# cityflow-project/CityFlow

Measured on NVIDIA H100. Metric: vehicle_steps_per_sec, higher is better.
Workload: dtype f64

## Files before the change

### cityflow_b200/csrc/device_phases_a.cuh

```cuda
#pragma once

namespace cfb {

__device__ __forceinline__ void blkSet(const View &V, int slot, int val) {
    if (val == -2) {
        V.blk[slot] = -1;
        V.delStep[slot] = V.ctrl->step;
    } else {
        V.blk[slot] = val;
    }
    if (V.blkUpd) {
        const int i = atomicAdd(&V.ctrl->nBlkUpd, 1);
        if (i < V.blkUpdCap) V.blkUpd[1 + i] = make_int2(slot, val); else atomicOr(&V.ctrl->error, ERR_MOVER_OVERFLOW);
    }
}

__device__ __forceinline__ int planAt(const View &V, int plan, int idx) { return V.planData[V.planBeg[plan] + idx]; }
__device__ __forceinline__ void foeTerms(const View &V, Notify &n, int foeLinkW);

__device__ void headSearch(const View &V, int d, double dis, int nextDrv, int planIdx, const DTmpl &T, int myLane,
                           int &outLeader, double &outGap) {
    int leader = -1;
    double gap = 0;
    double x = V.drvLength[d] - dis;
    int nd = nextDrv;
    for (int i = 0;; ++i) {
        if (i > 0) nd = V.planData[planIdx + 1 + i];
        if (nd < 0) break;
        if (nd >= V.nLanes) {
            const int sl = V.llStartLane[nd - V.nLanes];
            for (int q = V.laneOutBeg[sl]; q < V.laneOutBeg[sl + 1]; ++q) {
                const Tail t = V.tail[V.nLanes + V.laneOutLinks[q]];
                if (t.pos >= 0) {
                    double candGap = x + t.dis - t.len;
                    if (leader < 0 || candGap < gap) {
                        leader = t.pos;
                        gap = candGap;
                    }
                }
            }
            if (leader >= 0) break;
        } else {
            Tail t = V.tail[nd];
            if (myLane >= 0 && nd > myLane && (V.inserted[nd] & 1)) {
                const int c = V.count[nd] - 1;
                if (c > 0) {
                    const int tp = V.off[nd] + c - 1;
                    t.pos = tp;
                    t.dis = V.kin[tp].x;
                    t.len = V.tmpl[V.ids[tp].y].len;
                } else {
                    t.pos = -1;
                }
            }
            if (t.pos >= 0) {
                leader = t.pos;
                gap = x + t.dis - t.len;
                break;
            }
        }
        x += V.drvLength[nd];
        if (x > T.approachDist) break;
    }
    outLeader = leader;
    if (leader >= 0) outGap = gap;
}

// ... 177 lines not shown
        }
        if (valid && owner >= 0) {
            Notify n;
            n.dist = ndist;
            n.pos = owner;
            n.epoch = epoch;
            foeTerms(V, n, linkW);
            V.notify[V.lcIdx[cb + k]] = n;
            const int peer = V.lcPeer[cb + k];
            const int foeLink = V.csLink[V.lcIdx[cb + k] ^ 1];
            const int bit = peer - V.llCrossBeg[foeLink];
            atomicOr(&V.foeMask[foeLink * V.maskWords + (bit >> 5)], 1u << (bit & 31));
        }
    }
}

__device__ __forceinline__ void phase_notify(const View &V, const int bid, const int nblk) {
    const int lane = threadIdx.x & 31, tile = lane >> 4, tl = lane & 15;
    const int warp = (bid * blockDim.x + threadIdx.x) >> 5;
    const int nWarps = (nblk * blockDim.x) >> 5;
    const int cpar = V.par;
    const int nAct = V.ctrl->nAct[cpar];
    const int epoch = V.ctrl->step + 1;
    for (int w0 = 2 * warp; w0 < nAct; w0 += 2 * nWarps) {
        const int w = w0 + tile;
        int la = -1, lb = -1;
        if (w < nAct) {
            const int d = V.actList[cpar][w];
            if (d >= V.nLanes) {
                la = d - V.nLanes;
            } else if (V.count[d] > 0) {
                const int c = V.count[d], base = V.off[d];
                if ((V.inserted[d] & 2) && tl == 0 && !V.lcOn) {
                    const int4 idv = V.ids[base];
                    int ld = -1;
                    double g = 0;
                    headSearch(V, d, 0.0, idv.w, V.nav[base].x, V.tmpl[idv.y], d, ld, g);
                    V.leader[base] = ld;
                    if (ld >= 0) V.gap[base] = g;
                    if (V.lcOn && ld >= 0) V.lc.slot[idv.x].gap = g;
                }
                const int prev = V.nav[base + c - 1].y;
                if (prev >= V.nLanes && V.count[prev] == 0 && (!V.owned || V.owned[prev] == 1)) la = prev - V.nLanes;
                const int nx = V.ids[base].w;
                if (nx >= V.nLanes && V.count[nx] == 0 && nx - V.nLanes != la) lb = nx - V.nLanes;
                if (la < 0) { la = lb; lb = -1; }
            }
        }
        notifyLink(V, la, tl, epoch);
        if (__ballot_sync(0xffffffffu, lb >= 0)) notifyLink(V, lb, tl, epoch);
    }
    for (int w0 = 2 * warp; w0 < V.nBoundOut; w0 += 2 * nWarps) {
        const int w = w0 + tile;
        int l = -1;
        if (w < V.nBoundOut) {
            const Tail t = V.tail[V.boundOut[w]];
            if (t.pos >= 0 && t.prev >= V.nLanes && V.owned[t.prev] == 1 && V.count[t.prev] == 0) l = t.prev - V.nLanes;
        }
        notifyLink(V, l, tl, epoch);
    }
}

}
```

### cityflow_b200/csrc/device_phases_b.cuh

```cuda
#pragma once

namespace cfb {

static_assert(ENT_CAP <= 16, "k_move sorts a drivable's entrants inside one 16-lane tile");
__device__ __forceinline__ void phase_move(const View &V, const int bid, const int nblk) {
    const int lane = threadIdx.x & 31, tile = lane >> 4, tl = lane & 15, tb = lane & 16;
    const int cpar = V.par, npar = cpar ^ 1;
    const int nAct = V.ctrl->nAct[cpar];
    const int nTot = nAct + V.ctrl->nExtra;
    __shared__ int sTot[16];
    __shared__ int sBaseVeh, sBaseAct;
    const int tib = threadIdx.x >> 4, tpb = blockDim.x >> 4;
    for (int w0 = bid * tpb; w0 < nTot; w0 += nblk * tpb) {
        const int w = w0 + tib;
        int d = -1, n = 0, mIn = 0, base = 0, cap = 0;
        if (w < nTot) {
            d = w < nAct ? V.actList[cpar][w] : V.extraList[w - nAct];
            n = V.count[d];
            mIn = V.entCnt[d];
            base = V.off[d];
            cap = V.off[d + 1] - base;
        }
        const int nMax = max(n, __shfl_xor_sync(0xffffffffu, n, 16));
        int nsurv = 0;
// ... 115 lines not shown
            }
            V.tail[d] = t;
        }
        if (tl == 0) sTot[tib] = total;
        __syncthreads();
        if (threadIdx.x == 0) {
            int sv = 0, sa = 0;
            for (int k = 0; k < tpb; ++k) { sv += sTot[k]; sa += sTot[k] > 0; }
            sBaseVeh = sv ? atomicAdd(&V.ctrl->nVeh[npar], sv) : 0;
            sBaseAct = sa ? atomicAdd(&V.ctrl->nAct[npar], sa) : 0;
        }
        __syncthreads();
        if (total > 0) {
            int offV = sBaseVeh, offA = sBaseAct;
            for (int k = 0; k < tib; ++k) { offV += sTot[k]; offA += sTot[k] > 0; }
            if (tl == 0) V.actList[npar][offA] = d;
            for (int k = tl; k < total; k += 16)
                if (offV + k < V.vehCap) V.vehList[npar][offV + k] = make_int2(base + k, k == 0 ? (d | HEAD_BIT) : d);
        }
        __syncthreads();
    }
}

__device__ __forceinline__ void phase_leader(const View &V, const int bid, const int nblk) {
    const int gtid = bid * blockDim.x + threadIdx.x;
    const int lane = threadIdx.x & 31;
    const int warp = gtid >> 5;
    const int nWarps = (nblk * blockDim.x) >> 5;
    const int npar = V.par ^ 1;
    const int nAct = V.ctrl->nAct[npar];
    if (gtid == 0) {
        V.ctrl->step += 1;
        V.ctrl->epoch += 1;
        V.ctrl->vehicleSteps += (unsigned long long) (long long) V.ctrl->active;
        if (V.hostMirror) {
            volatile int *m = V.hostMirror;
            m[1] = V.ctrl->active;
            m[2] = V.ctrl->error;
            m[3] = V.ctrl->ties;
            __threadfence_system();
            m[0] = V.ctrl->epoch;
        }
    }
    if (!V.rl) {
        for (int in = gtid; in < V.nInter; in += nblk * blockDim.x) {
            if (V.interVirtual[in]) continue;
            double rem = V.remain[in] - V.dt;
            int cur = V.curPhase[in];
            const int pb = V.interPhaseBeg[in], nph = V.interPhaseBeg[in + 1] - pb;
            while (rem <= 0.0) {
                cur = (cur + 1) % nph;
                rem += V.phaseTime[pb + cur];
            }
            V.remain[in] = rem;
            V.curPhase[in] = cur;
        }
    }
    const int stride = nblk * blockDim.x;
    (void) lane; (void) warp; (void) nWarps;
    for (int w = gtid; w < nAct; w += stride) {
        const int d = V.actList[npar][w];
        const int p = V.off[d];
        const int4 idv = V.ids[p];
        int ld = -1;
        double g = 0;
        headSearch(V, d, V.kin[p].x, idv.w, V.nav[p].x, V.tmpl[idv.y], -1, ld, g);
        V.leader[p] = ld;
        if (ld >= 0) V.gap[p] = g;
        if (V.lcOn && ld >= 0) V.lc.slot[idv.x].gap = g;
    }
}

}
```

### cityflow_b200/csrc/device_sim.cu

```cuda
#include <cuda_runtime.h>
#include <cooperative_groups.h>

#include <algorithm>
#include <chrono>
#include <climits>
#include <cstdio>
#include <cstdlib>
#include <cstring>
#include <stdexcept>
#include <string>
#include <vector>

#include "device_sim.h"
#include "partition.h"
#include "shard.h"

namespace cfb {
namespace cg = cooperative_groups;

#define CFB_CUDA(x)                                                                                  \
    do {                                                                                             \
        cudaError_t e_ = (x);                                                                        \
        if (e_ != cudaSuccess)                                                                       \
            throw std::runtime_error(std::string("cityflow_b200 CUDA error: ") + cudaGetErrorString(e_) + \
// ... 4 lines not shown
#include "device_view.cuh"
#include "device_image.cuh"
#include "device_layout.cuh"
#include "device_phases_a.cuh"
namespace cfb {
__device__ __forceinline__ void pdlEnter() {
    asm volatile("griddepcontrol.wait;" ::: "memory");
    asm volatile("griddepcontrol.launch_dependents;" ::: "memory");
}
__global__ void __launch_bounds__(256) k_ingest(View V) { pdlEnter(); phase_ingest(V, blockIdx.x, gridDim.x); }
__global__ void __launch_bounds__(256) k_notify(View V) { pdlEnter(); phase_notify(V, blockIdx.x, gridDim.x); }

}
#include "device_control.cuh"
namespace cfb {

__global__ void __launch_bounds__(256, 4) k_control(View V) { pdlEnter(); phase_control(V, blockIdx.x, gridDim.x); }

}
#include "device_phases_b.cuh"
namespace cfb {
__global__ void __launch_bounds__(256) k_move(View V) { pdlEnter(); phase_move(V, blockIdx.x, gridDim.x); }
__global__ void __launch_bounds__(256) k_leader(View V) { pdlEnter(); phase_leader(V, blockIdx.x, gridDim.x); }

__global__ void __launch_bounds__(256, 4) k_step(View V) {
    cg::grid_group grid = cg::this_grid();
    phase_ingest(V, blockIdx.x, gridDim.x);
    grid.sync();
    phase_notify(V, blockIdx.x, gridDim.x);
    grid.sync();
    phase_control(V, blockIdx.x, gridDim.x);
    grid.sync();
    phase_move(V, blockIdx.x, gridDim.x);
    grid.sync();
    phase_leader(V, blockIdx.x, gridDim.x);
}

}
#include "device_shard.cuh"
namespace cfb {

__global__ void k_mask_counts(View V, int *out) {
    const int i = blockIdx.x * blockDim.x + threadIdx.x;
    if (i == 0) out[0] = V.ctrl->active;
    if (i < V.nLanes) out[1 + i] = (!V.owned || V.owned[i] == 1) ? V.count[i] : 0;
}
// ... 228 lines not shown
    cudaEvent_t obsReady = nullptr, obsConsumed = nullptr;
    cudaEvent_t actReady = nullptr, actTaken = nullptr;
    bool hPhaseStale = false;
    std::vector<cudaEvent_t> stepEv;
    size_t stepEvUsed = 0;
    DevBuf<unsigned char> flushBuf;
    KernelTimes times;
    cudaEvent_t shardEv[SHARD_PHASES + 1] = {};
    double shardMs[SHARD_PHASES] = {};
    long long shardTimedSteps = 0;

    DevBuf<LcSlot> lcSlot;
    DevBuf<int> lcLaneRoad, lcRouteLastRoad, lcScratch;
    bool lcSerial = false;
    DevBuf<int> lcSegIdx, lcPosDrv, lcSegBeg, lcLaneIdx, lcLaneRoadN, lcPlanRoute, lcPlanRoadPos, lcLanePlanRoad,
        lcLanePlanBeg, lcLanePlanId, lcCand, lcInvolved, lcSpare, lcPrio;
    DevBuf<double> lcSegStart, lcLaneWidth;
    DevBuf<int2> lcShadowLog;
    DevBuf<LcCtrl> lcCtrl;
    LcCtrl *hLcCtrl = nullptr;
    int lcSpareCap = 0;
    int slotCap = 0;
    int numSMs = 132;
    int gridNotify = 0, gridMove = 0, gridLeader = 0, gridControl = 0;
    bool mirrorStale = false;
    bool usePdl = true;
    bool useGraph = true, useCoop = false;
    GraphRing graphs;
    int gridStep = 0;
    int lastForm[4] = {};

    void invalidateGraphs() {
        graphs.drop(stream);
        shardGraphs.drop(stream);
    }
    void ensureGrids() {
        if (gridNotify) return;
        int b = 0;
        CFB_CUDA(cudaOccupancyMaxActiveBlocksPerMultiprocessor(&b, k_notify, 256, 0)); gridNotify = std::max(b, 1) * numSMs;
        CFB_CUDA(cudaOccupancyMaxActiveBlocksPerMultiprocessor(&b, k_move, 256, 0)); gridMove = std::max(b, 1) * numSMs;
        CFB_CUDA(cudaOccupancyMaxActiveBlocksPerMultiprocessor(&b, k_leader, 256, 0)); gridLeader = std::max(b, 1) * numSMs;
        CFB_CUDA(cudaOccupancyMaxActiveBlocksPerMultiprocessor(&b, k_control, 256, 0)); gridControl = std::max(b, 1) * numSMs;
    }
    enum StepKernel { INGEST, NOTIFY, CONTROL, MOVE, LEADER };
    void launchStep(StepKernel k, bool pdl) {
        static void (*const kernel[5])(View) = {k_ingest, k_notify, k_control, k_move, k_leader};
        ensureGrids();
        const int TPB = 256;
        const int ingest = (V.ingLanes ? std::max(std::max(V.nIngLanes, V.nIngRL), V.nIngLinks * V.maskWords / 4)
                                       : std::max(V.nLanes, V.nRL)) + TPB - 1;
        const int grid[5] = {std::max(ingest / TPB, 1), gridNotify, gridControl, gridMove, gridLeader};
        launchPdl(kernel[k], grid[k], TPB, stream, pdl && k != INGEST, V);
    }
    bool pdl() const { return usePdl && !timing; }

    void shardTimeMark(int k) {
        if (!shardEv[k]) CFB_CUDA(cudaEventCreate(&shardEv[k]));
        CFB_CUDA(cudaEventRecord(shardEv[k], stream));
    }
    void shardTimeCollect() {
        CFB_CUDA(cudaEventSynchronize(shardEv[SHARD_PHASES]));
        for (int k = 0; k < SHARD_PHASES; ++k) {
            float ms = 0;
            cudaEventElapsedTime(&ms, shardEv[k], shardEv[k + 1]);
            shardMs[k] += ms;
        }
        shardTimedSteps += 1;
    }
    static int moverGrid(int lanes) { return std::max(1, std::min(64, (lanes * 32 + 127) / 128)); }
    static constexpr int TAIL_GRID = 16;
    void launchSeam(void (*k)(View, ShardP2P), int grid) { launchPdl(k, grid, 128, stream, pdl(), V, S); }
    void shardSegment(int k, bool marks, long long &launches) {
        auto mark = [&](int e) { if (marks) shardTimeMark(e); };
        if (k == 0) {
            mark(0);
            launchStep(INGEST, false);
            mark(1);
// ... 96 lines not shown
    }
};

DeviceSim::DeviceSim(const RoadNet &net, const std::vector<VehicleTemplate> &templates, const Routing &routing,
                     const DeviceSimOptions &opt)
    : impl_(new Impl()) {
    Impl &I = *impl_;
    I.opt = opt;
    int ndev = 0;
    cudaError_t e = cudaGetDeviceCount(&ndev);
    if (e != cudaSuccess || ndev == 0) {
        delete impl_;
        impl_ = nullptr;
        throw std::runtime_error(std::string("cityflow_b200: no CUDA device available (") +
                                 (e != cudaSuccess ? cudaGetErrorString(e) : "device count 0") +
                                 "); this engine has no CPU fallback");
    }
    CFB_CUDA(cudaSetDevice(opt.device));
    CFB_CUDA(cudaStreamCreateWithFlags(&I.stream, cudaStreamNonBlocking));
    CFB_CUDA(cudaDeviceGetAttribute(&I.numSMs, cudaDevAttrMultiProcessorCount, opt.device));
    if (const char *g = getenv("CITYFLOW_B200_NO_GRAPH")) I.useGraph = !(g[0] == '1');
    if (const char *g = getenv("CITYFLOW_B200_COOP")) I.useCoop = (g[0] == '1');
    if (const char *g = getenv("CITYFLOW_B200_NO_PDL")) I.usePdl = !(g[0] == '1');
    {
        int coop = 0;
        cudaDeviceGetAttribute(&coop, cudaDevAttrCooperativeLaunch, opt.device);
        if (!coop) I.useCoop = false;
    }
    View &V = I.V;
    V.dt = opt.interval;
    V.rl = opt.rlTrafficLight ? 1 : 0;

    I.L = deviceLayout(net, V, cfb::bucketSpacing(templates));
    const DeviceLayout &L = I.L;
    const int nL = V.nLanes, nK = V.nLinks, nD = V.nDrv;
    I.P = L.P;
    I.drvLength.upload(L.drvLength); I.drvMaxSpeed.upload(L.drvMaxSpeed); I.off.upload(L.off);
    I.laneOutBeg.upload(L.laneOutBeg); I.laneOutLinks.upload(L.laneOutLinks);
    I.llStartLane.upload(L.llStartLane); I.llEndLane.upload(L.llEndLane); I.llRoadLink.upload(L.llRoadLink);
    I.linkInfo.upload(L.linkInfo);
    I.llCrossBeg.upload(L.llCrossBeg); I.lcIdx.upload(L.lcIdx); I.lcDist.upload(L.lcDist); I.lcPeer.upload(L.lcPeer); I.csLink.upload(L.csLink);
    I.interPhaseBeg.upload(L.interPhaseBeg); I.interRLBeg.upload(L.interRLBeg);
    I.phaseAvailBeg.upload(L.phaseAvailBeg); I.rlInter.upload(L.rlInter);
    I.phaseTime.upload(L.phaseTime); I.phaseAvail.upload(L.phaseAvail); I.interVirtual.upload(L.interVirtual);

    V.drvLength = I.drvLength.p; V.drvMaxSpeed = I.drvMaxSpeed.p; V.off = I.off.p;
// ... 5 lines not shown

    uploadTemplates(templates);
    uploadPlans(routing);

    const size_t P = (size_t) I.P;
    I.kin.alloc(P); I.nkin.alloc(P); I.gap.alloc(P); I.leader.alloc(P); I.ids.alloc(P); I.nav.alloc(P); I.nbuf.alloc(P);
    I.count.alloc(nD); I.entCnt.alloc(nD); I.ent.alloc((size_t) nD * ENT_CAP);
    I.waitHead.alloc(std::max(nL, 1)); I.waitTail.alloc(std::max(nL, 1)); I.inserted.alloc(std::max(nL, 1));
    I.notify.alloc(std::max(2 * net.nCross(), 1));
    I.curPhase.alloc(net.nInter()); I.remain.alloc(net.nInter()); I.rlAvail.alloc(std::max(net.nRoadLinks(), 1));
    I.mkin.alloc(V.moverCap); I.mids.alloc(V.moverCap); I.mnav.alloc(V.moverCap);
    I.cust.alloc(P); V.cust = I.cust.p;
    I.tail.alloc(nD); I.foeMask.alloc((size_t) std::max(nK, 1) * V.maskWords);
    V.tail = I.tail.p; V.foeMask = I.foeMask.p;
#ifdef CFB_DEBUG_COUNTERS
    I.dbgCyc.alloc(P); I.dbgPath.alloc(P); I.dbgCyc.fill(0); I.dbgPath.fill(0);
    V.dbgCyc = I.dbgCyc.p; V.dbgPath = I.dbgPath.p;
#endif
    I.vehList0.alloc(P); I.vehList1.alloc(P); I.act0.alloc(nD); I.act1.alloc(nD); I.extra.alloc(nD);
    V.vehList[0] = I.vehList0.p; V.vehList[1] = I.vehList1.p; V.actList[0] = I.act0.p; V.actList[1] = I.act1.p;
    V.extraList = I.extra.p;
    I.finSlots.alloc(V.finCap);
    I.ctrl.alloc(1);
    CFB_CUDA(cudaMallocHost(&I.hCtrl, sizeof(Ctrl)));
    {
        int *hm = nullptr, *dm = nullptr;
        CFB_CUDA(cudaHostAlloc(&hm, 64, cudaHostAllocMapped));
        memset(hm, 0, 64);
        CFB_CUDA(cudaHostGetDevicePointer(&dm, hm, 0));
        I.hMirror = hm;
        V.hostMirror = dm;
        if (const char *g = getenv("CITYFLOW_B200_NO_MIRROR")) if (g[0] == '1') V.hostMirror = nullptr;
        I.lastForm[3] = V.hostMirror != nullptr;
    }
    V.kin = I.kin.p; V.nkin = I.nkin.p; V.gap = I.gap.p; V.leader = I.leader.p; V.ids = I.ids.p; V.nav = I.nav.p;
    V.nbuf = I.nbuf.p; V.count = I.count.p; V.entCnt = I.entCnt.p; V.ent = I.ent.p;
    V.waitHead = I.waitHead.p; V.waitTail = I.waitTail.p; V.inserted = I.inserted.p; V.notify = I.notify.p;
    V.curPhase = I.curPhase.p; V.remain = I.remain.p; V.rlAvail = I.rlAvail.p;
    V.mkin = I.mkin.p; V.mids = I.mids.p; V.mnav = I.mnav.p; V.finSlots = I.finSlots.p; V.ctrl = I.ctrl.p;
    ensureSlotCapacity(opt.slotCapacity);
    for (int r = 0; r < Impl::RING; ++r) CFB_CUDA(cudaEventCreateWithFlags(&I.spawnDone[r], cudaEventDisableTiming));
    for (auto &ev : I.ev) CFB_CUDA(cudaEventCreate(&ev));
    reset();
}

DeviceSim::~DeviceSim() {
// ... 76 lines not shown
        nlc.fill(0);
        if (I.slotCap) CFB_CUDA(cudaMemcpy(nlc.p, I.lcSlot.p, I.slotCap * sizeof(LcSlot), cudaMemcpyDeviceToDevice));
        std::swap(I.lcSlot.p, nlc.p); std::swap(I.lcSlot.n, nlc.n);
        I.V.lc.slot = I.lcSlot.p;
    }
    legacySync();
    I.slotCap = cap;
    I.V.pos = I.pos.p; I.V.waitNext = I.waitNext.p; I.V.slotInfo = I.slotInfo.p; I.V.slotCust = I.slotCust.p; I.V.blk = I.blk.p; I.V.delStep = I.delStep.p;
    I.invalidateGraphs();
}

void DeviceSim::reset() {
    Impl &I = *impl_;
    CFB_CUDA(cudaStreamSynchronize(I.stream));
    applyFills(resetFills(I.V, (size_t) I.P, (size_t) I.slotCap));
    CFB_CUDA(cudaMemcpy(I.remain.p, I.L.remain0.data(), I.L.remain0.size() * sizeof(double), cudaMemcpyHostToDevice));
    I.hPhase.assign(I.V.nInter, 0);
    I.phaseDirty = false;
    I.hPhaseStale = false;
    if (I.hMirror) { I.hMirror[1] = 0; I.hMirror[2] = 0; I.hMirror[3] = 0; }
    I.mirrorStale = false;
    steps_ = 0;
    legacySync();
}

int DeviceSim::numPositions() const { return impl_->P; }
int DeviceSim::numDrivables() const { return impl_->V.nDrv; }
int DeviceSim::device() const { return impl_->opt.device; }

void DeviceSim::stageStep(const SpawnRec *recs, int n) {
    Impl &I = *impl_;
    View &V = I.V;
    cudaStream_t s = I.stream;
    if (n + 1 > I.spawnCap) {
        CFB_CUDA(cudaStreamSynchronize(s));
        I.spawnCap = std::max(1024, (n + 1) * 2);
        I.spawn.alloc(I.spawnCap);
        I.invalidateGraphs();
    }
    V.spawn = I.spawn.p + 1;
    const int r = I.ringIdx;
    I.ringIdx = (I.ringIdx + 1) % Impl::RING;
    CFB_CUDA(cudaEventSynchronize(I.spawnDone[r]));
    if (n + 1 > I.hSpawnCap[r]) {
        if (I.hSpawn[r]) cudaFreeHost(I.hSpawn[r]);
        I.hSpawnCap[r] = std::max(1024, (n + 1) * 2);
        CFB_CUDA(cudaMallocHost(&I.hSpawn[r], I.hSpawnCap[r] * sizeof(SpawnRec)));
    }
    if (I.phaseDirty) {
        if (!I.hPhaseRing[r]) CFB_CUDA(cudaMallocHost(&I.hPhaseRing[r], std::max(V.nInter, 1) * sizeof(int)));
        memcpy(I.hPhaseRing[r], I.hPhase.data(), V.nInter * sizeof(int));
        CFB_CUDA(cudaMemcpyAsync(V.curPhase, I.hPhaseRing[r], V.nInter * sizeof(int), cudaMemcpyHostToDevice, s));
        I.phaseDirty = false;
    }
    I.hSpawn[r][0].slot = n;
    if (n > 0) memcpy(I.hSpawn[r] + 1, recs, n * sizeof(SpawnRec));
    CFB_CUDA(cudaMemcpyAsync(I.spawn.p, I.hSpawn[r], (size_t) (n + 1) * sizeof(SpawnRec), cudaMemcpyHostToDevice, s));
    CFB_CUDA(cudaEventRecord(I.spawnDone[r], s));
    V.par = (int) (steps_ & 1);
}

void DeviceSim::step(const SpawnRec *recs, int n) {
    stageStep(recs, n);
    Impl &I = *impl_;
    View &V = I.V;
    cudaStream_t s = I.stream;
    I.ensureGrids();
    const bool tm = I.timing;
    auto launchAll = [&]() {
        for (int k = 0; k < 5; ++k) {
            if (tm) cudaEventRecord(I.ev[k], s);
            I.launchStep((Impl::StepKernel) k, I.pdl());
        }
        if (tm) cudaEventRecord(I.ev[5], s);
    };
    if (!tm && I.useCoop) {
        if (!I.gridStep) {
            int b = 0;
            CFB_CUDA(cudaOccupancyMaxActiveBlocksPerMultiprocessor(&b, k_step, 256, 0));
            I.gridStep = std::max(b, 1) * I.numSMs;
        }
        void *args[] = {(void *) &V};
        CFB_CUDA(cudaLaunchCooperativeKernel((void *) k_step, dim3(I.gridStep), dim3(256), args, 0, s));
    } else if (tm || !I.useGraph) {
        launchAll();
    } else {
        GraphRing &G = I.graphs;
        const int r = GraphRing::slot(steps_);
        cudaGraphExec_t &ge = G.exec[V.par][r];
        cudaGraph_t &g = G.tmpl[V.par];
        for (int attempt = 0; attempt < 2 && !ge; ++attempt) {
            if (!g) {
                CFB_CUDA(cudaStreamBeginCapture(s, cudaStreamCaptureModeThreadLocal));
                launchAll();
                if (cudaStreamEndCapture(s, &g) != cudaSuccess) g = nullptr;
            }
            if (!g || !G.instantiate(V.par, r)) {
                cudaGetLastError();
                if (g) { cudaGraphDestroy(g); g = nullptr; }
                ge = nullptr;
                if (!I.usePdl) throw std::runtime_error("cityflow_b200: cannot capture the step into a CUDA graph");
                I.usePdl = false;
            }
        }
        if (G.busy(V.par, r)) launchAll();
        else G.launch(V.par, r, s);
    }
    CFB_CUDA(cudaGetLastError());
    {
        const bool coop = !tm && I.useCoop;
        I.lastForm[0] = !tm && !coop && I.useGraph;
        I.lastForm[1] = !tm && !coop && I.usePdl;
        I.lastForm[2] = coop;
        I.lastForm[3] = V.hostMirror != nullptr;
    }
    launches_ += (!tm && I.useCoop) ? 1 : 5;
    steps_ += 1;
    I.epochHost += 1;
    I.mirrorStale = false;
    if (tm) {
        CFB_CUDA(cudaEventSynchronize(I.ev[5]));
        float ms[5];
        for (int k = 0; k < 5; ++k) cudaEventElapsedTime(&ms[k], I.ev[k], I.ev[k + 1]);
        I.times.ingest += ms[0]; I.times.notify += ms[1]; I.times.control += ms[2]; I.times.move += ms[3];
        I.times.leader += ms[4];
        I.times.launches += 1;
    }
}

static void readCtrlImpl(cudaStream_t s, Ctrl *dst, const Ctrl *src);
void DeviceSim::synchronize() { CFB_CUDA(cudaStreamSynchronize(impl_->stream)); }

void DeviceSim::configureShard(int rank, int world, const std::vector<unsigned char> &owned,
                               const std::vector<std::vector<int>> &feedPerPeer,
                               const std::vector<std::vector<int>> &ownPerPeer,
                               const std::vector<std::vector<int>> &boundarySize,
                               const std::vector<unsigned char> &ownedRoadLinks) {
    Impl &I = *impl_;
    View &V = I.V;
// ... 21 lines not shown
    I.blkAll.alloc((size_t) world * (1 + V.blkUpdCap));
    I.blkUpd.fill(0); I.blkAll.fill(0);
    V.blkUpd = I.blkUpd.p;
    I.useGraph = false;
    I.useCoop = false;
    if (const char *g = getenv("CITYFLOW_B200_SHARD_GRAPH")) I.shardGraphOk = (g[0] != '0');
    legacySync();
}

ShardBuffers DeviceSim::shardBuffers() {
    Impl &I = *impl_;
    ShardBuffers b;
    b.stream = (void *) I.stream;
    b.tailSend = I.tailSend.p; b.tailRecv = I.tailRecv.p; b.moverSend = I.moverSend.p; b.moverRecv = I.moverRecv.p;
    b.tailBytes = sizeof(TailMsg); b.moverBytes = sizeof(MoverMsg);
    b.outBeg = I.outBeg; b.inBeg = I.inBeg;
    b.blkSend = I.blkUpd.p; b.blkAll = I.blkAll.p;
    b.blkBytesPerRank = (size_t) (1 + I.V.blkUpdCap) * sizeof(int2);
    return b;
}

void DeviceSim::shardStep(const SpawnRec *recs, int n, ShardTransport *t) {
    Impl &I = *impl_;
    stageStep(recs, n);
    for (int attempt = 0; attempt < 2; ++attempt) {
        const int st = I.shardGraphBegin(steps_);
        if (st != 1) try {
            I.shardKernels(t, launches_);
        } catch (const std::exception &) {
            if (st != 2 || I.p2p) throw;
        }
        if (I.shardGraphEnd(st, steps_)) break;
    }
    CFB_CUDA(cudaGetLastError());
    steps_ += 1;
    I.epochHost += 1;
}

void DeviceSim::shardSegment(int k) {
    Impl &I = *impl_;
    I.shardSegment(k, false, launches_);
    if (k == 2) {
        CFB_CUDA(cudaGetLastError());
        steps_ += 1;
        I.epochHost += 1;
    }
// ... 323 lines not shown
    slots.resize(n);
    if (n > 0) {
        CFB_CUDA(cudaMemcpyAsync(slots.data(), I.finSlots.p, n * sizeof(int2), cudaMemcpyDeviceToHost, I.stream));
        CFB_CUDA(cudaMemsetAsync(&I.V.ctrl->finCount, 0, sizeof(int), I.stream));
        CFB_CUDA(cudaStreamSynchronize(I.stream));
    }
    return n;
}

void DeviceSim::phases(int32_t *out) {
    Impl &I = *impl_;
    if (I.V.rl && !I.hPhaseStale) { memcpy(out, I.hPhase.data(), I.V.nInter * sizeof(int)); return; }
    CFB_CUDA(cudaMemcpyAsync(out, I.V.curPhase, I.V.nInter * sizeof(int), cudaMemcpyDeviceToHost, I.stream));
    CFB_CUDA(cudaStreamSynchronize(I.stream));
    if (I.V.rl) {
        I.hPhase.assign(out, out + I.V.nInter);
        I.hPhaseStale = false;
    }
}

int DeviceSim::leaderSlotOf(int slot) {
    Impl &I = *impl_;
    if (slot < 0 || slot >= I.slotCap) return -2;
    int p = -1;
    CFB_CUDA(cudaMemcpyAsync(&p, I.V.pos + slot, sizeof(int), cudaMemcpyDeviceToHost, I.stream));
    CFB_CUDA(cudaStreamSynchronize(I.stream));
    if (p < 0) return -2;
    int lp = -1;
    CFB_CUDA(cudaMemcpy(&lp, I.V.leader + p, sizeof(int), cudaMemcpyDeviceToHost));
    if (lp < 0) return -1;
    int4 idv;
    CFB_CUDA(cudaMemcpy(&idv, I.V.ids + lp, sizeof(int4), cudaMemcpyDeviceToHost));
    return idv.x;
}

void DeviceSim::laneVehicleSlots(std::vector<int32_t> &slots, std::vector<int32_t> &laneBeg) {
    Impl &I = *impl_;
    const int nL = I.V.nLanes;
    std::vector<int32_t> cnt(nL);
    laneVehicleCount(cnt.data());
    laneBeg.assign(nL + 1, 0);
    for (int l = 0; l < nL; ++l) laneBeg[l + 1] = laneBeg[l] + cnt[l];
    slots.resize(laneBeg[nL]);
    if (slots.empty()) return;
    DevBuf<int> dBeg, dOut;
    dBeg.upload(std::vector<int>(laneBeg.begin(), laneBeg.end()));
    dOut.alloc(slots.size());
    const int TPB = 256;
    k_lane_slots<<<(nL * 32 + TPB - 1) / TPB, TPB, 0, I.stream>>>(I.V, dOut.p, dBeg.p);
    CFB_CUDA(cudaMemcpyAsync(slots.data(), dOut.p, slots.size() * sizeof(int), cudaMemcpyDeviceToHost, I.stream));
    CFB_CUDA(cudaStreamSynchronize(I.stream));
    launches_ += 1;
}

struct HostDump {
    std::vector<int> count, leader, del;
    std::vector<double2> kin;
    std::vector<double> gap;
    std::vector<int4> ids, nav;
    std::vector<LcSlot> lc;
    View V{};
};
template <class T> static void copyDown(std::vector<T> &dst, const T *src, size_t n) {
    dst.resize(n);
    if (n) CFB_CUDA(cudaMemcpy(dst.data(), src, n * sizeof(T), cudaMemcpyDeviceToHost));
}
static void dumpToHost(DeviceSim::Impl &I, HostDump &h, bool withLc) {
    CFB_CUDA(cudaStreamSynchronize(I.stream));
    const size_t P = (size_t) I.P;
    copyDown(h.del, I.V.delStep, (size_t) I.slotCap);
    readCtrlImpl(I.stream, I.hCtrl, I.V.ctrl);
    copyDown(h.count, I.V.count, (size_t) I.V.nDrv);
    copyDown(h.leader, I.V.leader, P);
    copyDown(h.kin, I.V.kin, P);
    copyDown(h.ids, I.V.ids, P);
    copyDown(h.nav, I.V.nav, P);
    if (withLc) copyDown(h.lc, I.lcSlot.p, (size_t) I.slotCap);
    else copyDown(h.gap, I.V.gap, P);
    View &V = h.V;
    V.nDrv = I.V.nDrv;
    V.off = I.L.off.data(); V.count = h.count.data(); V.leader = h.leader.data(); V.kin = h.kin.data(); V.gap = h.gap.data();
    V.ids = h.ids.data(); V.nav = h.nav.data(); V.delStep = h.del.data(); V.ctrl = I.hCtrl; V.lc.slot = h.lc.data();
}

void DeviceSim::debugDump(std::vector<DebugRec> &out) {
    HostDump h;
    dumpToHost(*impl_, h, false);
    debugRecords(h.V, impl_->ownedHost.empty() ? nullptr : impl_->ownedHost.data(), out);
}

struct DeviceSim::Snapshot {
    ImageHeader h;
    DevBuf<unsigned char> blob;
};

static std::vector<std::pair<void *, size_t>> snapshotRegions(DeviceSim::Impl &I) {
    return snapshotRegions(I.V, (size_t) I.P, (size_t) I.slotCap);
}

DeviceSim::Snapshot *DeviceSim::snapshot() {
    Impl &I = *impl_;
    CFB_CUDA(cudaStreamSynchronize(I.stream));
    if (I.phaseDirty && I.V.nInter) {
        CFB_CUDA(cudaMemcpyAsync(I.V.curPhase, I.hPhase.data(), I.V.nInter * sizeof(int), cudaMemcpyHostToDevice, I.stream));
        CFB_CUDA(cudaStreamSynchronize(I.stream));
        I.phaseDirty = false;
    }
    auto regs = snapshotRegions(I);
    Snapshot *s = new Snapshot();
    s->h = imageHeader(steps_, I.slotCap, regs);
    s->blob.alloc(s->h.payload());
    size_t off = 0;
    for (auto &r : regs) {
        if (r.second) CFB_CUDA(cudaMemcpyAsync(s->blob.p + off, r.first, r.second, cudaMemcpyDeviceToDevice, I.stream));
        off += imagePad(r.second);
    }
    CFB_CUDA(cudaStreamSynchronize(I.stream));
    return s;
}

void DeviceSim::restore(const Snapshot *s) {
    Impl &I = *impl_;
    ensureSlotCapacity(s->h.slotCap);
    CFB_CUDA(cudaStreamSynchronize(I.stream));
    auto regs = snapshotRegions(I);
    checkImageFits(s->h, regs, I.V);
    applyFills(slotFills(I.V, (size_t) I.slotCap));
    legacySync();
    size_t off = 0;
    for (size_t k = 0; k < regs.size(); ++k) {
        const size_t bytes = s->h.regions[k];
        if (bytes) CFB_CUDA(cudaMemcpyAsync(regs[k].first, s->blob.p + off, bytes, cudaMemcpyDeviceToDevice, I.stream));
        off += imagePad(bytes);
    }
    I.hPhase.resize(I.V.nInter);
    if (I.V.nInter) {
        CFB_CUDA(cudaMemcpyAsync(I.hPhase.data(), I.V.curPhase, I.V.nInter * sizeof(int), cudaMemcpyDeviceToHost, I.stream));
        CFB_CUDA(cudaStreamSynchronize(I.stream));
    }
    I.phaseDirty = false;
    I.hPhaseStale = false;
    {
        readCtrlImpl(I.stream, I.hCtrl, I.V.ctrl);
        I.epochHost = I.hCtrl->epoch;
        if (I.hMirror) { I.hMirror[1] = I.hCtrl->active; I.hMirror[2] = I.hCtrl->error; I.hMirror[3] = I.hCtrl->ties; I.hMirror[0] = I.hCtrl->epoch; }
        I.mirrorStale = false;
    }
    applyFills(scratchFills(I.V));
    CFB_CUDA(cudaStreamSynchronize(I.stream));
    legacySync();
    steps_ = s->h.steps;
}

void DeviceSim::freeSnapshot(Snapshot *s) { delete s; }

static ImageGeometry imageGeometry(DeviceSim::Impl &I) {
    return ImageGeometry{I.L.off.data(), I.V.nDrv, I.V.nLanes, I.V.nInter, (size_t) I.P};
}
void DeviceSim::decodeSnapshot(const Snapshot *s, StateImage &out) {
    std::vector<unsigned char> blob;
    snapshotToHost(s, blob);
    decodeImage(blob, imageGeometry(*impl_), out);
}
DeviceSim::Snapshot *DeviceSim::encodeSnapshot(const StateImage &in) {
    std::vector<unsigned char> blob;
    encodeImage(in, imageGeometry(*impl_), blob);
    return snapshotFromHost(blob.data(), blob.size());
}

// ... 45 lines not shown
    out.speed = k.y;
    return true;
}

void DeviceSim::setCustomSpeed(int slot, double speed) {
    Impl &I = *impl_;
    CFB_CUDA(cudaStreamSynchronize(I.stream));
    int p = -1;
    CFB_CUDA(cudaMemcpy(&p, I.V.pos + slot, sizeof(int), cudaMemcpyDeviceToHost));
    double *dst = p >= 0 ? I.V.cust + p : I.V.slotCust + slot;
    double old = 0;
    CFB_CUDA(cudaMemcpy(&old, dst, sizeof(double), cudaMemcpyDeviceToHost));
    CFB_CUDA(cudaMemcpy(dst, &speed, sizeof(double), cudaMemcpyHostToDevice));
    if (old != old) {
        readCtrlImpl(I.stream, I.hCtrl, I.V.ctrl);
        int n = I.hCtrl->nCustom + 1;
        CFB_CUDA(cudaMemcpy(&I.V.ctrl->nCustom, &n, sizeof(int), cudaMemcpyHostToDevice));
    }
    legacySync();
}

void DeviceSim::setVehiclePlan(int slot, int planId, int planIdx, int nextDrv) {
    Impl &I = *impl_;
    CFB_CUDA(cudaStreamSynchronize(I.stream));
    int p = -1;
    CFB_CUDA(cudaMemcpy(&p, I.V.pos + slot, sizeof(int), cudaMemcpyDeviceToHost));
    if (p >= 0) {
        CFB_CUDA(cudaMemcpy(&I.V.nav[p].x, &planIdx, sizeof(int), cudaMemcpyHostToDevice));
        CFB_CUDA(cudaMemcpy(&I.V.ids[p].w, &nextDrv, sizeof(int), cudaMemcpyHostToDevice));
    } else {
        CFB_CUDA(cudaMemcpy(&I.V.slotInfo[slot].z, &planId, sizeof(int), cudaMemcpyHostToDevice));
    }
    legacySync();
}

void DeviceSim::setPhase(int intersection, int phase) {
    Impl &I = *impl_;
    if (I.hPhaseStale) {
        CFB_CUDA(cudaMemcpyAsync(I.hPhase.data(), I.V.curPhase, I.V.nInter * sizeof(int), cudaMemcpyDeviceToHost, I.stream));
        CFB_CUDA(cudaStreamSynchronize(I.stream));
        I.hPhaseStale = false;
    }
    I.hPhase[intersection] = phase;
    I.phaseDirty = true;
}

// ... 20 lines not shown
    V.lc.laneRoad = I.lcLaneRoad.p;
    I.lcSegIdx.alloc(I.P); I.lcSegIdx.fill(0);
    I.lcCand.alloc(LC_MAX_CAND); I.lcInvolved.alloc(LC_MAX_CAND); I.lcShadowLog.alloc(LC_MAX_CAND); I.lcPrio.alloc(LC_MAX_CAND);
    I.lcCtrl.alloc(1); I.lcCtrl.fill(0);
    I.lcScratch.alloc((size_t) 4 * LC_MAX_CAND); I.lcScratch.fill(0);
    if (const char *g = getenv("CITYFLOW_B200_LC_SERIAL")) I.lcSerial = g[0] == '1';
    I.lcSlot.alloc(std::max(I.slotCap, 1)); I.lcSlot.fill(0);
    CFB_CUDA(cudaMallocHost(&I.hLcCtrl, sizeof(LcCtrl)));
    LcView &C = V.lc;
    C.slot = I.lcSlot.p; C.segIdx = I.lcSegIdx.p; C.posDrv = I.lcPosDrv.p; C.segBeg = I.lcSegBeg.p; C.segStart = I.lcSegStart.p;
    C.laneIdx = I.lcLaneIdx.p; C.laneRoadN = I.lcLaneRoadN.p; C.laneWidth = I.lcLaneWidth.p;
    C.cand = I.lcCand.p; C.involved = I.lcInvolved.p; C.shadowLog = I.lcShadowLog.p; C.ctrl = I.lcCtrl.p;
    C.scratchA = I.lcScratch.p; C.scratchB = I.lcScratch.p + LC_MAX_CAND; C.scratchC = I.lcScratch.p + 2 * LC_MAX_CAND;
    C.scratchD = I.lcScratch.p + 3 * LC_MAX_CAND;
    C.spare = nullptr; C.nSpare = 0;
    V.lcOn = 1;
    I.useGraph = false;
    I.useCoop = false;
    legacySync();
    uploadLanePlans(routing);
}

void DeviceSim::stepLcBegin(const SpawnRec *recs, int n, const int32_t *spare, int nSpare, std::vector<LcShadow> &created) {
    stageStep(recs, n);
    Impl &I = *impl_;
    View &V = I.V;
    cudaStream_t s = I.stream;
    const int TPB = 256;
    I.ensureGrids();
    if (nSpare > I.lcSpareCap) {
        CFB_CUDA(cudaStreamSynchronize(s));
        I.lcSpareCap = std::max(1024, nSpare * 2);
        I.lcSpare.alloc(I.lcSpareCap);
    }
    if (nSpare > 0) CFB_CUDA(cudaMemcpyAsync(I.lcSpare.p, spare, nSpare * sizeof(int), cudaMemcpyHostToDevice, s));
    V.lc.spare = I.lcSpare.p;
    V.lc.nSpare = nSpare;
    k_lc_begin<<<1, 1, 0, s>>>(V.lc);
    I.launchStep(Impl::INGEST, false);
    k_lc_admitted<<<I.gridNotify, TPB, 0, s>>>(V, V.lc);
    k_lc_segments<<<I.gridNotify, TPB, 0, s>>>(V, V.lc);
    k_lc_signal<<<I.gridControl, TPB, 0, s>>>(V, V.lc);
    if (I.lcSerial) {
        k_lc_schedule<<<1, 32, 0, s>>>(V, V.lc);
    } else {
        k_lc_order<<<1, 256, 0, s>>>(V, V.lc);
        k_lc_schedule_roads<<<LC_MAX_CAND / 128, 128, 0, s>>>(V, V.lc);
        k_lc_log<<<1, 32, 0, s>>>(V, V.lc);
// ... 21 lines not shown
        CFB_CUDA(cudaMemcpyAsync(I.lcPrio.p, priorities, n * sizeof(int), cudaMemcpyHostToDevice, s));
        k_lc_priorities<<<(n + 127) / 128, 128, 0, s>>>(V, V.lc, I.lcPrio.p, n);
    }
    k_lc_leader<<<I.gridNotify, TPB, 0, s>>>(V, V.lc);
    I.launchStep(Impl::NOTIFY, false);
    I.launchStep(Impl::CONTROL, false);
    if (I.lcSerial) {
        k_lc_control_tail<<<1, 32, 0, s>>>(V, V.lc);
    } else {
        k_lc_tail_order<<<1, 256, 0, s>>>(V, V.lc);
        k_lc_tail_roads<<<LC_MAX_CAND / 128, 128, 0, s>>>(V, V.lc);
        k_lc_tail_clear<<<1, 32, 0, s>>>(V, V.lc);
    }
    I.launchStep(Impl::MOVE, false);
    I.launchStep(Impl::LEADER, false);
    CFB_CUDA(cudaGetLastError());
    launches_ += 6 + (n > 0);
    steps_ += 1;
    I.epochHost += 1;
}

void DeviceSim::debugDumpLc(std::vector<LcDebugRec> &out) {
    HostDump h;
    dumpToHost(*impl_, h, true);
    lcDebugRecords(h.V, out);
}

}
```

### cityflow_b200/csrc/device_view.cuh

```cuda
#pragma once

namespace cfb {

struct DTmpl {
    double len, maxPosAcc, maxNegAcc, usualPosAcc, usualNegAcc, minGap, maxSpeed, headwayTime;
    double yieldDistance, turnSpeed, approachDist, speed0, pad[4];
};

struct __align__(16) Notify {
    double dist;
    int pos;
    int epoch;
    int slot, prio, enterLL, steps;
    int flags;
    int pad0, pad1, pad2;
};
constexpr int NF_CAN_YIELD = 1;
constexpr int NF_PASSED = 2;
constexpr int NF_CYCLE = 4;

struct __align__(16) Tail {
    double dis, len, speed;
    int pos, prev;
};
// ... 65 lines not shown
    unsigned char *rlAvail;
    int *entCnt, *ent;
    double2 *mkin;
    int4 *mids, *mnav;
    int2 *finSlots;
    int2 *vehList[2];
    int *actList[2];
    int *extraList;
    double *cust;
    double *slotCust;
    int *blk;
    int *delStep;
    const unsigned char *owned;
    const int *ingLanes, *ingLinks, *ingRL;
    int nIngLanes, nIngLinks, nIngRL;
    const int *boundOut;
    const int *boundIn;
    int nBoundOut, nBoundIn;
    int2 *blkUpd;
    int blkUpdCap;
    unsigned *dbgCyc, *dbgPath;
    Ctrl *ctrl;
    int *hostMirror;
    const SpawnRec *spawn;
    int lcOn;
    LcView lc;
};

__device__ __forceinline__ double min2(double x, double y) { return x < y ? x : y; }
__device__ __forceinline__ double max2(double x, double y) { return x > y ? x : y; }
__device__ __forceinline__ int x86int(double x) {
    return (x > -2147483649.0 && x < 2147483648.0) ? (int) x : INT_MIN;
}
constexpr double kEps = 1e-8;

__device__ __forceinline__ double noCollisionSpeed(double vL, double dL, double vF, double dF, double gap, double dt,
                                                   double targetGap) {
    double c = vF * dt / 2 + targetGap - 0.5 * vL * vL / dL - gap;
    double a = 0.5 / dF;
    double b = 0.5 * dt;
    if (b * b < 4 * a * c) return -100;
    double v1 = 0.5 / a * (sqrt(b * b - 4 * a * c) - b);
    double v2 = 2 * vL - dL * dt + 2 * (gap - targetGap) / dt;
    return min2(v1, v2);
}
__device__ __forceinline__ double stopBeforeSpeed(const DTmpl &T, double speed, double distance, double dt) {
// ... 27 lines not shown
```

Measured before the change: 1.449 billion.

## Fold leader kernel into notify and move kernels, four launches per step

```diff
diff --git a/cityflow_b200/csrc/device_phases_a.cuh b/cityflow_b200/csrc/device_phases_a.cuh
--- a/cityflow_b200/csrc/device_phases_a.cuh
+++ b/cityflow_b200/csrc/device_phases_a.cuh
@@ -18,6 +18,7 @@
 __device__ __forceinline__ int planAt(const View &V, int plan, int idx) { return V.planData[V.planBeg[plan] + idx]; }
 __device__ __forceinline__ void foeTerms(const View &V, Notify &n, int foeLinkW);
 
+constexpr int UNDO_ADMISSIONS = -2;
 __device__ void headSearch(const View &V, int d, double dis, int nextDrv, int planIdx, const DTmpl &T, int myLane,
                            int &outLeader, double &outGap) {
     int leader = -1;
@@ -42,7 +43,7 @@
             if (leader >= 0) break;
         } else {
             Tail t = V.tail[nd];
-            if (myLane >= 0 && nd > myLane && (V.inserted[nd] & 1)) {
+            if (myLane != -1 && nd > myLane && (V.inserted[nd] & 1)) {
                 const int c = V.count[nd] - 1;
                 if (c > 0) {
                     const int tp = V.off[nd] + c - 1;
@@ -266,24 +267,27 @@
     const int cpar = V.par;
     const int nAct = V.ctrl->nAct[cpar];
     const int epoch = V.ctrl->step + 1;
+    const bool heads = V.fourKernel && V.fourKernel[0] != V.ctrl->step && !V.lcOn;
     for (int w0 = 2 * warp; w0 < nAct; w0 += 2 * nWarps) {
         const int w = w0 + tile;
         int la = -1, lb = -1;
         if (w < nAct) {
             const int d = V.actList[cpar][w];
+            const bool admitted = d < V.nLanes && (V.inserted[d] & 2) && !V.lcOn;
+            if ((admitted || heads) && tl == 0 && V.count[d] > 0) {
+                const int base = V.off[d];
+                const int4 idv = V.ids[base];
+                int ld = -1;
+                double g = 0;
+                headSearch(V, d, admitted ? 0.0 : V.kin[base].x, idv.w, V.nav[base].x, V.tmpl[idv.y], admitted ? d : UNDO_ADMISSIONS,
+                           ld, g);
+                V.leader[base] = ld;
+                if (ld >= 0) V.gap[base] = g;
+            }
             if (d >= V.nLanes) {
                 la = d - V.nLanes;
             } else if (V.count[d] > 0) {
                 const int c = V.count[d], base = V.off[d];
-                if ((V.inserted[d] & 2) && tl == 0 && !V.lcOn) {
-                    const int4 idv = V.ids[base];
-                    int ld = -1;
-                    double g = 0;
-                    headSearch(V, d, 0.0, idv.w, V.nav[base].x, V.tmpl[idv.y], d, ld, g);
-                    V.leader[base] = ld;
-                    if (ld >= 0) V.gap[base] = g;
-                    if (V.lcOn && ld >= 0) V.lc.slot[idv.x].gap = g;
-                }
                 const int prev = V.nav[base + c - 1].y;
                 if (prev >= V.nLanes && V.count[prev] == 0 && (!V.owned || V.owned[prev] == 1)) la = prev - V.nLanes;
                 const int nx = V.ids[base].w;
diff --git a/cityflow_b200/csrc/device_phases_b.cuh b/cityflow_b200/csrc/device_phases_b.cuh
--- a/cityflow_b200/csrc/device_phases_b.cuh
+++ b/cityflow_b200/csrc/device_phases_b.cuh
@@ -161,42 +161,42 @@
     }
 }
 
-__device__ __forceinline__ void phase_leader(const View &V, const int bid, const int nblk) {
-    const int gtid = bid * blockDim.x + threadIdx.x;
-    const int lane = threadIdx.x & 31;
-    const int warp = gtid >> 5;
-    const int nWarps = (nblk * blockDim.x) >> 5;
+__device__ __forceinline__ void stepEnd(const View &V) {
+    volatile Ctrl *c = V.ctrl;
+    const int step = c->step, epoch = c->epoch, active = c->active, error = c->error, ties = c->ties;
+    const unsigned long long vs = c->vehicleSteps;
+    c->step = step + 1;
+    c->epoch = epoch + 1;
+    c->vehicleSteps = vs + (unsigned long long) (long long) active;
+    if (V.hostMirror) {
+        volatile int *m = V.hostMirror;
+        m[1] = active;
+        m[2] = error;
+        m[3] = ties;
+        __threadfence_system();
+        m[0] = epoch + 1;
+    }
+}
+
+__device__ __forceinline__ void passTime(const View &V, const int gtid, const int stride) {
+    if (V.rl) return;
+    for (int in = gtid; in < V.nInter; in += stride) {
+        if (V.interVirtual[in]) continue;
+        double rem = V.remain[in] - V.dt;
+        int cur = V.curPhase[in];
+        const int pb = V.interPhaseBeg[in], nph = V.interPhaseBeg[in + 1] - pb;
+        while (rem <= 0.0) {
+            cur = (cur + 1) % nph;
+            rem += V.phaseTime[pb + cur];
+        }
+        V.remain[in] = rem;
+        V.curPhase[in] = cur;
+    }
+}
+
+__device__ __forceinline__ void searchHeads(const View &V, const int gtid, const int stride) {
     const int npar = V.par ^ 1;
     const int nAct = V.ctrl->nAct[npar];
-    if (gtid == 0) {
-        V.ctrl->step += 1;
-        V.ctrl->epoch += 1;
-        V.ctrl->vehicleSteps += (unsigned long long) (long long) V.ctrl->active;
-        if (V.hostMirror) {
-            volatile int *m = V.hostMirror;
-            m[1] = V.ctrl->active;
-            m[2] = V.ctrl->error;
-            m[3] = V.ctrl->ties;
-            __threadfence_system();
-            m[0] = V.ctrl->epoch;
-        }
-    }
-    if (!V.rl) {
-        for (int in = gtid; in < V.nInter; in += nblk * blockDim.x) {
-            if (V.interVirtual[in]) continue;
-            double rem = V.remain[in] - V.dt;
-            int cur = V.curPhase[in];
-            const int pb = V.interPhaseBeg[in], nph = V.interPhaseBeg[in + 1] - pb;
-            while (rem <= 0.0) {
-                cur = (cur + 1) % nph;
-                rem += V.phaseTime[pb + cur];
-            }
-            V.remain[in] = rem;
-            V.curPhase[in] = cur;
-        }
-    }
-    const int stride = nblk * blockDim.x;
-    (void) lane; (void) warp; (void) nWarps;
     for (int w = gtid; w < nAct; w += stride) {
         const int d = V.actList[npar][w];
         const int p = V.off[d];
@@ -210,4 +210,35 @@
     }
 }
 
-}
+__device__ __forceinline__ void phase_leader(const View &V, const int bid, const int nblk) {
+    const int gtid = bid * blockDim.x + threadIdx.x;
+    const int stride = nblk * blockDim.x;
+    if (gtid == 0) stepEnd(V);
+    passTime(V, gtid, stride);
+    searchHeads(V, gtid, stride);
+}
+
+__device__ __forceinline__ void phase_lights(const View &V, const int bid, const int nblk) {
+    passTime(V, bid * blockDim.x + threadIdx.x, nblk * blockDim.x);
+}
+__device__ __forceinline__ void phase_move_end(const View &V, const int bid, const int nblk) {
+    phase_move(V, bid, nblk);
+    __shared__ int sLast;
+    __threadfence();
+    __syncthreads();
+    if (threadIdx.x == 0) sLast = atomicAdd(&V.fourKernel[1], 1) == nblk - 1;
+    __syncthreads();
+    if (sLast && threadIdx.x == 0) {
+        V.fourKernel[1] = 0;
+        __threadfence();
+        stepEnd(V);
+    }
+}
+
+__device__ __forceinline__ void phase_heads(const View &V, const int bid, const int nblk) {
+    const int gtid = bid * blockDim.x + threadIdx.x;
+    searchHeads(V, gtid, nblk * blockDim.x);
+    if (gtid == 0) V.fourKernel[0] = V.ctrl->step;
+}
+
+}
diff --git a/cityflow_b200/csrc/device_sim.cu b/cityflow_b200/csrc/device_sim.cu
--- a/cityflow_b200/csrc/device_sim.cu
+++ b/cityflow_b200/csrc/device_sim.cu
@@ -50,6 +50,12 @@
 namespace cfb {
 __global__ void __launch_bounds__(256) k_move(View V) { pdlEnter(); phase_move(V, blockIdx.x, gridDim.x); }
 __global__ void __launch_bounds__(256) k_leader(View V) { pdlEnter(); phase_leader(V, blockIdx.x, gridDim.x); }
+__global__ void __launch_bounds__(256) k_move_end(View V) {
+    phase_lights(V, blockIdx.x, gridDim.x);
+    pdlEnter();
+    phase_move_end(V, blockIdx.x, gridDim.x);
+}
+__global__ void __launch_bounds__(256) k_heads(View V) { phase_heads(V, blockIdx.x, gridDim.x); }
 
 __global__ void __launch_bounds__(256, 4) k_step(View V) {
     cg::grid_group grid = cg::this_grid();
@@ -324,10 +330,13 @@
     int lcSpareCap = 0;
     int slotCap = 0;
     int numSMs = 132;
-    int gridNotify = 0, gridMove = 0, gridLeader = 0, gridControl = 0;
+    int gridNotify = 0, gridMove = 0, gridLeader = 0, gridControl = 0, gridMoveEnd = 0;
     bool mirrorStale = false;
     bool usePdl = true;
     bool useGraph = true, useCoop = false;
+    bool leaderKernel = false;
+    DevBuf<int> fourKernel;
+    bool headsPending = false;
     GraphRing graphs;
     int gridStep = 0;
     int lastForm[4] = {};
@@ -343,18 +352,39 @@
         CFB_CUDA(cudaOccupancyMaxActiveBlocksPerMultiprocessor(&b, k_move, 256, 0)); gridMove = std::max(b, 1) * numSMs;
         CFB_CUDA(cudaOccupancyMaxActiveBlocksPerMultiprocessor(&b, k_leader, 256, 0)); gridLeader = std::max(b, 1) * numSMs;
         CFB_CUDA(cudaOccupancyMaxActiveBlocksPerMultiprocessor(&b, k_control, 256, 0)); gridControl = std::max(b, 1) * numSMs;
+        CFB_CUDA(cudaOccupancyMaxActiveBlocksPerMultiprocessor(&b, k_move_end, 256, 0)); gridMoveEnd = std::max(b, 1) * numSMs;
     }
     enum StepKernel { INGEST, NOTIFY, CONTROL, MOVE, LEADER };
-    void launchStep(StepKernel k, bool pdl) {
+    void launchStep(StepKernel k, bool pdl, bool four = false) {
         static void (*const kernel[5])(View) = {k_ingest, k_notify, k_control, k_move, k_leader};
         ensureGrids();
         const int TPB = 256;
         const int ingest = (V.ingLanes ? std::max(std::max(V.nIngLanes, V.nIngRL), V.nIngLinks * V.maskWords / 4)
                                        : std::max(V.nLanes, V.nRL)) + TPB - 1;
         const int grid[5] = {std::max(ingest / TPB, 1), gridNotify, gridControl, gridMove, gridLeader};
-        launchPdl(kernel[k], grid[k], TPB, stream, pdl && k != INGEST, V);
+        View v = V;
+        if (four) v.fourKernel = fourKernel.p;
+        if (four && k == MOVE) launchPdl(k_move_end, gridMoveEnd, TPB, stream, pdl, v);
+        else launchPdl(kernel[k], grid[k], TPB, stream, pdl && k != INGEST, v);
     }
     bool pdl() const { return usePdl && !timing; }
+    void settleHeads(long long &launches) {
+        if (!headsPending) return;
+        ensureGrids();
+        View v = V;
+        v.fourKernel = fourKernel.p;
+        v.par = V.par;
+        k_heads<<<gridLeader, 256, 0, stream>>>(v);
+        CFB_CUDA(cudaGetLastError());
+        headsPending = false;
+        launches += 1;
+    }
+    void stampHeads(int step) {
+        headsPending = false;
+        const int v[2] = {step, 0};
+        CFB_CUDA(cudaMemcpyAsync(fourKernel.p, v, sizeof(v), cudaMemcpyHostToDevice, stream));
+        CFB_CUDA(cudaStreamSynchronize(stream));
+    }
 
     void shardTimeMark(int k) {
         if (!shardEv[k]) CFB_CUDA(cudaEventCreate(&shardEv[k]));
@@ -497,6 +527,7 @@
     if (const char *g = getenv("CITYFLOW_B200_NO_GRAPH")) I.useGraph = !(g[0] == '1');
     if (const char *g = getenv("CITYFLOW_B200_COOP")) I.useCoop = (g[0] == '1');
     if (const char *g = getenv("CITYFLOW_B200_NO_PDL")) I.usePdl = !(g[0] == '1');
+    if (const char *g = getenv("CITYFLOW_B200_LEADER_KERNEL")) I.leaderKernel = (g[0] == '1');
     {
         int coop = 0;
         cudaDeviceGetAttribute(&coop, cudaDevAttrCooperativeLaunch, opt.device);
@@ -548,6 +579,7 @@
     V.extraList = I.extra.p;
     I.finSlots.alloc(V.finCap);
     I.ctrl.alloc(1);
+    I.fourKernel.alloc(2);
     CFB_CUDA(cudaMallocHost(&I.hCtrl, sizeof(Ctrl)));
     {
         int *hm = nullptr, *dm = nullptr;
@@ -670,6 +702,7 @@
     I.mirrorStale = false;
     steps_ = 0;
     legacySync();
+    I.stampHeads(0);
 }
 
 int DeviceSim::numPositions() const { return impl_->P; }
@@ -709,16 +742,19 @@
 }
 
 void DeviceSim::step(const SpawnRec *recs, int n) {
+    Impl &I = *impl_;
+    const bool tm = I.timing;
+    const bool four = !tm && !I.useCoop && !I.leaderKernel;
+    if (!four) I.settleHeads(launches_);
     stageStep(recs, n);
-    Impl &I = *impl_;
     View &V = I.V;
     cudaStream_t s = I.stream;
     I.ensureGrids();
-    const bool tm = I.timing;
+    const int nk = four ? 4 : 5;
     auto launchAll = [&]() {
-        for (int k = 0; k < 5; ++k) {
+        for (int k = 0; k < nk; ++k) {
             if (tm) cudaEventRecord(I.ev[k], s);
-            I.launchStep((Impl::StepKernel) k, I.pdl());
+            I.launchStep((Impl::StepKernel) k, I.pdl(), four);
         }
         if (tm) cudaEventRecord(I.ev[5], s);
     };
@@ -762,7 +798,8 @@
         I.lastForm[2] = coop;
         I.lastForm[3] = V.hostMirror != nullptr;
     }
-    launches_ += (!tm && I.useCoop) ? 1 : 5;
+    launches_ += (!tm && I.useCoop) ? 1 : nk;
+    I.headsPending = four;
     steps_ += 1;
     I.epochHost += 1;
     I.mirrorStale = false;
@@ -830,6 +867,7 @@
 
 void DeviceSim::shardStep(const SpawnRec *recs, int n, ShardTransport *t) {
     Impl &I = *impl_;
+    I.settleHeads(launches_);
     stageStep(recs, n);
     for (int attempt = 0; attempt < 2; ++attempt) {
         const int st = I.shardGraphBegin(steps_);
@@ -1199,6 +1237,7 @@
 int DeviceSim::leaderSlotOf(int slot) {
     Impl &I = *impl_;
     if (slot < 0 || slot >= I.slotCap) return -2;
+    I.settleHeads(launches_);
     int p = -1;
     CFB_CUDA(cudaMemcpyAsync(&p, I.V.pos + slot, sizeof(int), cudaMemcpyDeviceToHost, I.stream));
     CFB_CUDA(cudaStreamSynchronize(I.stream));
@@ -1242,7 +1281,8 @@
     dst.resize(n);
     if (n) CFB_CUDA(cudaMemcpy(dst.data(), src, n * sizeof(T), cudaMemcpyDeviceToHost));
 }
-static void dumpToHost(DeviceSim::Impl &I, HostDump &h, bool withLc) {
+static void dumpToHost(DeviceSim::Impl &I, HostDump &h, bool withLc, long long &launches) {
+    I.settleHeads(launches);
     CFB_CUDA(cudaStreamSynchronize(I.stream));
     const size_t P = (size_t) I.P;
     copyDown(h.del, I.V.delStep, (size_t) I.slotCap);
@@ -1262,7 +1302,7 @@
 
 void DeviceSim::debugDump(std::vector<DebugRec> &out) {
     HostDump h;
-    dumpToHost(*impl_, h, false);
+    dumpToHost(*impl_, h, false, launches_);
     debugRecords(h.V, impl_->ownedHost.empty() ? nullptr : impl_->ownedHost.data(), out);
 }
 
@@ -1277,6 +1317,7 @@
 
 DeviceSim::Snapshot *DeviceSim::snapshot() {
     Impl &I = *impl_;
+    I.settleHeads(launches_);
     CFB_CUDA(cudaStreamSynchronize(I.stream));
     if (I.phaseDirty && I.V.nInter) {
         CFB_CUDA(cudaMemcpyAsync(I.V.curPhase, I.hPhase.data(), I.V.nInter * sizeof(int), cudaMemcpyHostToDevice, I.stream));
@@ -1322,6 +1363,7 @@
         I.epochHost = I.hCtrl->epoch;
         if (I.hMirror) { I.hMirror[1] = I.hCtrl->active; I.hMirror[2] = I.hCtrl->error; I.hMirror[3] = I.hCtrl->ties; I.hMirror[0] = I.hCtrl->epoch; }
         I.mirrorStale = false;
+        I.stampHeads(I.hCtrl->step);
     }
     applyFills(scratchFills(I.V));
     CFB_CUDA(cudaStreamSynchronize(I.stream));
@@ -1413,6 +1455,7 @@
 
 void DeviceSim::setVehiclePlan(int slot, int planId, int planIdx, int nextDrv) {
     Impl &I = *impl_;
+    I.settleHeads(launches_);
     CFB_CUDA(cudaStreamSynchronize(I.stream));
     int p = -1;
     CFB_CUDA(cudaMemcpy(&p, I.V.pos + slot, sizeof(int), cudaMemcpyDeviceToHost));
@@ -1479,8 +1522,9 @@
 }
 
 void DeviceSim::stepLcBegin(const SpawnRec *recs, int n, const int32_t *spare, int nSpare, std::vector<LcShadow> &created) {
+    Impl &I = *impl_;
+    I.settleHeads(launches_);
     stageStep(recs, n);
-    Impl &I = *impl_;
     View &V = I.V;
     cudaStream_t s = I.stream;
     const int TPB = 256;
@@ -1548,7 +1592,7 @@
 
 void DeviceSim::debugDumpLc(std::vector<LcDebugRec> &out) {
     HostDump h;
-    dumpToHost(*impl_, h, true);
+    dumpToHost(*impl_, h, true, launches_);
     lcDebugRecords(h.V, out);
 }
 
diff --git a/cityflow_b200/csrc/device_view.cuh b/cityflow_b200/csrc/device_view.cuh
--- a/cityflow_b200/csrc/device_view.cuh
+++ b/cityflow_b200/csrc/device_view.cuh
@@ -111,6 +111,7 @@
     unsigned *dbgCyc, *dbgPath;
     Ctrl *ctrl;
     int *hostMirror;
+    int *fourKernel;
     const SpawnRec *spawn;
     int lcOn;
     LcView lc;
```

After: 1.508 billion, median of 6. 1.04x the previous value.
